# zyc00/Point-SAM

Hardware: NVIDIA H100
Metric: point-clouds/sec (N=32768, ViT-L, 512x64 groups) (higher is better)
Workload: dtype bf16x3

## Files before the change

point-sam_b200/csrc/attention_tc.cu:

```cuda
#include "psam_common.cuh"
#include "../../include/psam_b200.h"

namespace psam {

constexpr int ATT_BQ = 128;
constexpr int ATT_BKEY = 64;
constexpr int ATT_STAGES = 4;
constexpr int ATT_THREADS = 288;
constexpr int ATT_Q_TILE = 128 * 64 * 2;
constexpr int ATT_KV_TILE = 64 * 64 * 2;

template <int NCH>
struct AttSmem {
    static constexpr int Q = NCH * 2 * ATT_Q_TILE;
    static constexpr int STAGE = NCH * 2 * ATT_KV_TILE;
    static constexpr int TOTAL = Q + ATT_STAGES * STAGE + 1024;
};

struct AttnParams {
    int L, H, B;
    float scale_log2e;
    __nv_bfloat16* out_hi;
    long long out_plane, ldo, out_h, out_b;
};

__device__ __forceinline__ float ex2f(float x) {
    float e;
    asm("ex2.approx.ftz.f32 %0, %1;" : "=f"(e) : "f"(x));
    return e;
}

__device__ __forceinline__ float quad_max(float v) {
    v = fmaxf(v, __shfl_xor_sync(0xffffffffu, v, 1));
    return fmaxf(v, __shfl_xor_sync(0xffffffffu, v, 2));
}

__device__ __forceinline__ uint32_t bf16x2_bits(float lo, float hi) {
    const __nv_bfloat162 h2 = __floats2bfloat162_rn(lo, hi);
    return *reinterpret_cast<const uint32_t*>(&h2);
}

template <int NCH, int KS_LAST>
__device__ __forceinline__ void att_scores(float (&s)[32], uint32_t sq, uint32_t sk) {
#pragma unroll
    for (int i = 0; i < 32; ++i) s[i] = 0.f;
    fence_acc(s);
    wgmma_fence();
#pragma unroll
    for (int pass = 0; pass < 3; ++pass) {
#pragma unroll
        for (int ch = 0; ch < NCH; ++ch) {
            const uint64_t qd = gmma_desc_k(sq + ch * 2 * ATT_Q_TILE + (pass == 1 ? ATT_Q_TILE : 0));
            const uint64_t kd = gmma_desc_k(sk + ch * 2 * ATT_KV_TILE + (pass == 2 ? ATT_KV_TILE : 0));
#pragma unroll
            for (int k = 0; k < (ch == NCH - 1 ? KS_LAST : 4); ++k) wgmma_ss<64>(s, qd + 2 * k, kd + 2 * k, 1u);
        }
    }
    wgmma_commit();
    wgmma_wait<0>();
    fence_acc(s);
}

__device__ __forceinline__ void att_mask(float (&s)[32], int key0, int L, int lane) {
    if (key0 + ATT_BKEY <= L) return;
#pragma unroll
    for (int i = 0; i < 32; ++i)
        if (key0 + 8 * (i >> 2) + 2 * (lane & 3) + (i & 1) >= L) s[i] = __int_as_float(0xff800000);
}

template <int DH, bool TWO_PASS>
__global__ void __launch_bounds__(ATT_THREADS, 1)
attention_wgmma_kernel(const __grid_constant__ CUtensorMap tmap_q, const __grid_constant__ CUtensorMap tmap_k,
                       const __grid_constant__ CUtensorMap tmap_v, const AttnParams p) {
    constexpr int NCH = DH <= 64 ? 1 : 2;
    constexpr int KS_LAST = DH <= 64 ? 4 : (DH - 64 + 15) / 16;
    using S = AttSmem<NCH>;
    pdl_launch_dependents();
    extern __shared__ unsigned char smem_dyn[];
    __shared__ __align__(8) uint64_t q_full, kv_full[ATT_STAGES], kv_empty[ATT_STAGES];

    const uint32_t smem_base = (smem_u32(smem_dyn) + 1023u) & ~1023u;
    const uint32_t sQ = smem_base;
    const uint32_t sKV = sQ + S::Q;
    const int warp = threadIdx.x >> 5, lane = threadIdx.x & 31;
    const int q_tile = blockIdx.x, h = blockIdx.y, b = blockIdx.z;
    const int nkb = (p.L + ATT_BKEY - 1) / ATT_BKEY;

    if (warp == 8 && lane == 0) {
        tma_prefetch_desc(&tmap_q);
        tma_prefetch_desc(&tmap_k);
        tma_prefetch_desc(&tmap_v);
        mbar_init(smem_u32(&q_full), 1);
        for (int s = 0; s < ATT_STAGES; ++s) {
            mbar_init(smem_u32(&kv_full[s]), 1);
            mbar_init(smem_u32(&kv_empty[s]), 2);
        }
        fence_mbar_init();
    }
    __syncthreads();
    pdl_wait();

    const int n_items = (TWO_PASS ? 3 : 2) * nkb;
    if (warp == 8) {
        if (lane == 0) {
            const uint32_t qb = smem_u32(&q_full);
            mbar_arrive_expect_tx(qb, (uint32_t)S::Q);
            for (int ch = 0; ch < NCH; ++ch)
                tma_load_5d(sQ + ch * 2 * ATT_Q_TILE, &tmap_q, qb, 64 * ch, q_tile * ATT_BQ, 0, h, b);
            for (int i = 0; i < n_items; ++i) {
                const int s = i % ATT_STAGES;
                mbar_wait(smem_u32(&kv_empty[s]), ((uint32_t)(i / ATT_STAGES) & 1u) ^ 1u);
                const uint32_t fb = smem_u32(&kv_full[s]);
                mbar_arrive_expect_tx(fb, (uint32_t)S::STAGE);
                const int i2 = TWO_PASS ? i - nkb : i;
                const bool is_v = i2 >= 0 && (i2 & 1);
                const int blk = i2 < 0 ? i : (i2 >> 1);
                for (int ch = 0; ch < NCH; ++ch)
                    tma_load_5d(sKV + s * S::STAGE + ch * 2 * ATT_KV_TILE, is_v ? &tmap_v : &tmap_k, fb, 64 * ch, blk * ATT_BKEY, 0, h, b);
            }
        }
        return;
    }

    const int wg = warp >> 2;
    const bool leader = (warp & 3) == 0 && lane == 0;
    const uint32_t sq = sQ + wg * (ATT_Q_TILE / 2);
    const float c = p.scale_log2e;
    mbar_wait(smem_u32(&q_full), 0);
    int item = 0;
    auto acquire = [&]() {
        const int s = item % ATT_STAGES;
        mbar_wait(smem_u32(&kv_full[s]), (uint32_t)(item / ATT_STAGES) & 1u);
        return sKV + s * S::STAGE;
    };
    auto release = [&]() {
        if (leader) mbar_arrive(smem_u32(&kv_empty[item % ATT_STAGES]));
        ++item;
    };

    float m[2] = {__int_as_float(0xff800000), __int_as_float(0xff800000)};
    float s[32];
    if (TWO_PASS) {
        for (int j = 0; j < nkb; ++j) {
            att_scores<NCH, KS_LAST>(s, sq, acquire());
            release();
            att_mask(s, j * ATT_BKEY, p.L, lane);
#pragma unroll
            for (int i = 0; i < 32; ++i) m[(i >> 1) & 1] = fmaxf(m[(i >> 1) & 1], s[i]);
        }
        m[0] = quad_max(m[0]);
        m[1] = quad_max(m[1]);
    }
    float o[NCH][32];
#pragma unroll
    for (int ch = 0; ch < NCH; ++ch)
#pragma unroll
        for (int i = 0; i < 32; ++i) o[ch][i] = 0.f;
    float l[2] = {0.f, 0.f};
    for (int j = 0; j < nkb; ++j) {
        att_scores<NCH, KS_LAST>(s, sq, acquire());
        release();
        att_mask(s, j * ATT_BKEY, p.L, lane);
        if (!TWO_PASS) {
            float mb[2] = {m[0], m[1]};
#pragma unroll
            for (int i = 0; i < 32; ++i) mb[(i >> 1) & 1] = fmaxf(mb[(i >> 1) & 1], s[i]);
#pragma unroll
            for (int q = 0; q < 2; ++q) {
                mb[q] = quad_max(mb[q]);
                const float f = ex2f((m[q] - mb[q]) * c);
                l[q] *= f;
#pragma unroll
                for (int ch = 0; ch < NCH; ++ch)
#pragma unroll
                    for (int i = 0; i < 32; ++i)
                        if (((i >> 1) & 1) == q) o[ch][i] *= f;
                m[q] = mb[q];
            }
        }
        uint32_t ph[4][4], pl[4][4];
        const float nm[2] = {-m[0] * c, -m[1] * c};
#pragma unroll
        for (int kk = 0; kk < 4; ++kk) {
#pragma unroll
            for (int r = 0; r < 4; ++r) {
                const int i = 8 * kk + 2 * r, q = r & 1;
                const float e0 = ex2f(fmaf(s[i], c, nm[q])), e1 = ex2f(fmaf(s[i + 1], c, nm[q]));
                l[q] += e0 + e1;
                ph[kk][r] = bf16x2_bits(e0, e1);
                const float2 hf = __bfloat1622float2(*reinterpret_cast<const __nv_bfloat162*>(&ph[kk][r]));
                pl[kk][r] = bf16x2_bits(e0 - hf.x, e1 - hf.y);
            }
        }
        const uint32_t sv = acquire();
#pragma unroll
        for (int ch = 0; ch < NCH; ++ch) fence_acc(o[ch]);
        wgmma_fence();
#pragma unroll
        for (int ch = 0; ch < NCH; ++ch) {
            const uint64_t v_hi = gmma_desc_mn64(sv + ch * 2 * ATT_KV_TILE), v_lo = gmma_desc_mn64(sv + ch * 2 * ATT_KV_TILE + ATT_KV_TILE);
#pragma unroll
            for (int kk = 0; kk < 4; ++kk) {
                wgmma_rs_tb<64>(o[ch], ph[kk], v_hi + (uint64_t)(kk * (2048 >> 4)));
                wgmma_rs_tb<64>(o[ch], pl[kk], v_hi + (uint64_t)(kk * (2048 >> 4)));
                wgmma_rs_tb<64>(o[ch], ph[kk], v_lo + (uint64_t)(kk * (2048 >> 4)));
            }
        }
        wgmma_commit();
        wgmma_wait<0>();
#pragma unroll
        for (int ch = 0; ch < NCH; ++ch) fence_acc(o[ch]);
        release();
    }
    const int rbase = q_tile * ATT_BQ + wg * 64 + (warp & 3) * 16 + (lane >> 2);
#pragma unroll
    for (int q = 0; q < 2; ++q) {
        float lq = l[q] + __shfl_xor_sync(0xffffffffu, l[q], 1);
        lq += __shfl_xor_sync(0xffffffffu, lq, 2);
        const float inv = 1.0f / lq;
        const int row = rbase + 8 * q;
        if (row >= p.L) continue;
        __nv_bfloat16* ohi = p.out_hi + (long long)b * p.out_b + (long long)h * p.out_h + (long long)row * p.ldo;
        __nv_bfloat16* olo = ohi + p.out_plane;
#pragma unroll
        for (int ch = 0; ch < NCH; ++ch) {
#pragma unroll
            for (int g = 0; g < 8; ++g) {
                const int col = ch * 64 + 8 * g + 2 * (lane & 3);
                if (col >= DH) continue;
                __nv_bfloat16 h0, l0, h1, l1;
                split_bf16(o[ch][4 * g + 2 * q] * inv, h0, l0);
                split_bf16(o[ch][4 * g + 2 * q + 1] * inv, h1, l1);
                *reinterpret_cast<uint32_t*>(ohi + col) = pack_bf16x2(h0, h1);
                *reinterpret_cast<uint32_t*>(olo + col) = pack_bf16x2(l0, l1);
            }
        }
    }
}

int make_operand_map_ext(CUtensorMap* map, const psam_operand* op, int box_rows, int box_planes);

static int attention_setup(const psam_operand* q, const psam_operand* k, const psam_operand* v, void* out_hi, long long out_plane,
                           long long ldo, long long out_head_stride, long long out_cloud_stride, float scale, CUtensorMap* mq,
                           CUtensorMap* mk, CUtensorMap* mv, AttnParams* p, dim3* grid) {
    if (!q || !k || !v || !out_hi) return PSAM_ERR_ARG;
    const int L = q->rows, dh = q->k;
    const int H = q->nb1 > 0 ? q->nb1 : 1, B = q->nb2 > 0 ? q->nb2 : 1;
    if ((dh != 64 && dh != 88) || L <= 0) return PSAM_ERR_UNSUPPORTED;
    if (k->rows != L || v->rows != L || k->k != dh || v->k != dh) return PSAM_ERR_ARG;
    for (const psam_operand* x : {k, v})
        if ((x->nb1 > 0 ? x->nb1 : 1) != H || (x->nb2 > 0 ? x->nb2 : 1) != B) return PSAM_ERR_ARG;
    if (!(scale > 0.f) || !isfinite(scale)) return PSAM_ERR_ARG;
    if ((ldo | out_plane | out_head_stride | out_cloud_stride) & 7) return PSAM_ERR_ARG;
    int rc = make_operand_map_ext(mq, q, ATT_BQ, 2);
    if (rc) return rc;
    rc = make_operand_map_ext(mk, k, ATT_BKEY, 2);
    if (rc) return rc;
    rc = make_operand_map_ext(mv, v, ATT_BKEY, 2);
    if (rc) return rc;
    p->L = L, p->H = H, p->B = B;
    p->scale_log2e = scale * 1.4426950408889634f;
    p->out_hi = (__nv_bfloat16*)out_hi;
    p->out_plane = out_plane, p->ldo = ldo, p->out_h = out_head_stride, p->out_b = out_cloud_stride;
    *grid = dim3((unsigned)ceil_div(L, ATT_BQ), (unsigned)H, (unsigned)B);
    return PSAM_OK;
}

template <int DH, bool TWO_PASS>
static int launch_attention(const CUtensorMap& mq, const CUtensorMap& mk, const CUtensorMap& mv, const AttnParams& p, dim3 grid,
                            cudaStream_t stream) {
    auto kern = attention_wgmma_kernel<DH, TWO_PASS>;
    constexpr int smem = AttSmem<DH <= 64 ? 1 : 2>::TOTAL;
    PSAM_CUDA_TRY(cudaFuncSetAttribute(kern, cudaFuncAttributeMaxDynamicSharedMemorySize, smem));
    PSAM_CUDA_TRY(psam::launch(kern, grid, dim3(ATT_THREADS), (size_t)smem, stream, mq, mk, mv, p));
    PSAM_LAUNCH_CHECK();
    return PSAM_OK;
}

}

extern "C" int psam_attention_bf16x3(const psam_operand* q, const psam_operand* k, const psam_operand* v, void* out_hi,
                                     long long out_plane, long long ldo, long long out_head_stride,
                                     long long out_cloud_stride, float scale, cudaStream_t stream) {
    using namespace psam;
    CUtensorMap mq, mk, mv;
    AttnParams p;
    dim3 grid;
    int rc = attention_setup(q, k, v, out_hi, out_plane, ldo, out_head_stride, out_cloud_stride, scale, &mq, &mk, &mv, &p, &grid);
    if (rc) return rc;
    if (q->k == 88) return launch_attention<88, false>(mq, mk, mv, p, grid, stream);
    return launch_attention<64, false>(mq, mk, mv, p, grid, stream);
}

extern "C" int psam_attention_bf16x3_twopass(const psam_operand* q, const psam_operand* k, const psam_operand* v, void* out_hi,
                                             long long out_plane, long long ldo, long long out_head_stride,
                                             long long out_cloud_stride, float scale, cudaStream_t stream) {
    using namespace psam;
    CUtensorMap mq, mk, mv;
    AttnParams p;
    dim3 grid;
    if (q && q->k != 64) return PSAM_ERR_UNSUPPORTED;
    int rc = attention_setup(q, k, v, out_hi, out_plane, ldo, out_head_stride, out_cloud_stride, scale, &mq, &mk, &mv, &p, &grid);
    if (rc) return rc;
    return launch_attention<64, true>(mq, mk, mv, p, grid, stream);
}
```

point-sam_b200/csrc/psam_common.cuh:

```cuda
#pragma once
#include <cuda.h>
#include <cuda_bf16.h>
#include <cuda_runtime.h>
#include <stdint.h>
#include <stdlib.h>
#include <utility>

#define PSAM_OK 0
#define PSAM_ERR_ARG (-1)
#define PSAM_ERR_UNSUPPORTED (-2)

#define PSAM_CUDA_TRY(expr)                      \
    do {                                         \
        cudaError_t _e = (expr);                 \
        if (_e != cudaSuccess) return (int)_e;   \
    } while (0)

#define PSAM_LAUNCH_CHECK()                      \
    do {                                         \
        cudaError_t _e = cudaGetLastError();     \
        if (_e != cudaSuccess) return (int)_e;   \
    } while (0)

namespace psam {


__device__ __forceinline__ void pdl_launch_dependents() { asm volatile("griddepcontrol.launch_dependents;" ::: "memory"); }
__device__ __forceinline__ void pdl_wait() { asm volatile("griddepcontrol.wait;" ::: "memory"); }
__device__ __forceinline__ void pdl_prologue() {
    pdl_launch_dependents();
    pdl_wait();
}

inline bool pdl_enabled() {
    static int v = -1;
    if (v < 0) {
        const char* e = getenv("PSAM_PDL");
        v = (e && e[0] == '1') ? 1 : 0;
    }
    return v != 0;
}

template <typename... KArgs, typename... Args>
inline cudaError_t launch(void (*kernel)(KArgs...), dim3 grid, dim3 block, size_t smem, cudaStream_t stream, Args&&... args) {
    cudaLaunchConfig_t cfg = {};
    cfg.gridDim = grid;
    cfg.blockDim = block;
    cfg.dynamicSmemBytes = smem;
    cfg.stream = stream;
    cudaLaunchAttribute attr[1];
    attr[0].id = cudaLaunchAttributeProgrammaticStreamSerialization;
    attr[0].val.programmaticStreamSerializationAllowed = 1;
    cfg.attrs = attr;
    cfg.numAttrs = pdl_enabled() ? 1 : 0;
    return cudaLaunchKernelEx(&cfg, kernel, static_cast<KArgs>(std::forward<Args>(args))...);
}

__host__ __device__ inline int ceil_div(int a, int b) { return (a + b - 1) / b; }
__host__ __device__ inline long long ceil_div_ll(long long a, long long b) { return (a + b - 1) / b; }

__device__ __forceinline__ void split_bf16(float x, __nv_bfloat16& hi, __nv_bfloat16& lo) {
    hi = __float2bfloat16_rn(x);
    lo = __float2bfloat16_rn(x - __bfloat162float(hi));
}

__device__ __forceinline__ uint32_t pack_bf16x2(__nv_bfloat16 a, __nv_bfloat16 b) {
    return (uint32_t)__bfloat16_as_ushort(a) | ((uint32_t)__bfloat16_as_ushort(b) << 16);
}

__device__ __forceinline__ float gelu_erf(float x) {
    const float z = x * 0.70710678118654752440f;
    const float a = fabsf(z);
    const float t = __fdividef(1.0f, fmaf(0.3275911f, a, 1.0f));
    float p = fmaf(1.061405429f, t, -1.453152027f);
    p = fmaf(p, t, 1.421413741f);
    p = fmaf(p, t, -0.284496736f);
    p = fmaf(p, t, 0.254829592f);
    p *= t;
    const float e = __expf(-a * a);
    const float erf_abs = fmaf(-p, e, 1.0f);
    const float hx = 0.5f * x;
    return fmaf(hx, copysignf(erf_abs, z), hx);
}

__device__ __forceinline__ float silu(float x) { return x / (1.0f + __expf(-x)); }

__device__ __forceinline__ float sqdist3(float x, float y, float z, float cx, float cy, float cz) {
    const float dx = x - cx, dy = y - cy, dz = z - cz;
    return __fmaf_rn(dz, dz, __fmaf_rn(dy, dy, __fmul_rn(dx, dx)));
}

template <int NT>
__device__ __forceinline__ unsigned long long block_scan_u64(unsigned long long x, unsigned long long* sw, unsigned long long& total) {
    const int lane = threadIdx.x & 31, warp = threadIdx.x >> 5;
#pragma unroll
    for (int off = 1; off < 32; off <<= 1) {
        const unsigned long long y = __shfl_up_sync(0xffffffffu, x, off);
        if (lane >= off) x += y;
    }
    if (lane == 31) sw[warp] = x;
    __syncthreads();
    if (warp == 0) {
        unsigned long long s = lane < NT / 32 ? sw[lane] : 0ull;
#pragma unroll
        for (int off = 1; off < 32; off <<= 1) {
            const unsigned long long y = __shfl_up_sync(0xffffffffu, s, off);
            if (lane >= off) s += y;
        }
        sw[lane] = s;
    }
    __syncthreads();
    if (warp) x += sw[warp - 1];
    total = sw[NT / 32 - 1];
    __syncthreads();
    return x;
}

template <int NT>
__device__ __forceinline__ void scan_block_sums(unsigned long long* sums, int nb, unsigned long long* total) {
    __shared__ unsigned long long sw[32];
    unsigned long long carry = 0;
    for (int base = 0; base < nb; base += NT) {
        const int i = base + threadIdx.x;
        const unsigned long long v = i < nb ? sums[i] : 0ull;
        unsigned long long t;
        const unsigned long long x = block_scan_u64<NT>(v, sw, t);
        if (i < nb) sums[i] = carry + x - v;
        carry += t;
    }
    if (threadIdx.x == 0 && total) *total = carry;
}

enum Act { ACT_NONE = 0, ACT_GELU = 1, ACT_RELU = 2 };

__device__ __forceinline__ float apply_act(float x, int act) {
    if (act == ACT_GELU) return gelu_erf(x);
    if (act == ACT_RELU) return fmaxf(x, 0.0f);
    return x;
}

__device__ __forceinline__ uint32_t smem_u32(const void* p) {
    return (uint32_t)__cvta_generic_to_shared(p);
}

__device__ __forceinline__ void mbar_init(uint32_t bar, uint32_t count) {
    asm volatile("mbarrier.init.shared::cta.b64 [%0], %1;" ::"r"(bar), "r"(count));
}

__device__ __forceinline__ void fence_mbar_init() {
    asm volatile("fence.mbarrier_init.release.cluster;" ::: "memory");
}

__device__ __forceinline__ void fence_proxy_async() {
    asm volatile("fence.proxy.async.shared::cta;" ::: "memory");
}

__device__ __forceinline__ void mbar_arrive_expect_tx(uint32_t bar, uint32_t bytes) {
    asm volatile("mbarrier.arrive.expect_tx.shared::cta.b64 _, [%0], %1;" ::"r"(bar), "r"(bytes) : "memory");
}

__device__ __forceinline__ void mbar_arrive(uint32_t bar) {
    asm volatile("mbarrier.arrive.shared::cta.b64 _, [%0];" ::"r"(bar) : "memory");
}

__device__ __forceinline__ bool mbar_try_wait(uint32_t bar, uint32_t parity) {
    uint32_t ok;
    asm volatile(
        "{\n\t.reg .pred p;\n\t"
        "mbarrier.try_wait.parity.shared::cta.b64 p, [%1], %2;\n\t"
        "selp.b32 %0, 1, 0, p;\n\t}"
        : "=r"(ok)
        : "r"(bar), "r"(parity)
        : "memory");
    return ok != 0;
}

__device__ __forceinline__ void mbar_wait(uint32_t bar, uint32_t parity) {
    while (!mbar_try_wait(bar, parity)) {
    }
}

__device__ __forceinline__ void mbar_arrive_remote_release(uint32_t remote_bar) {
    asm volatile("mbarrier.arrive.release.cluster.shared::cluster.b64 _, [%0];" ::"r"(remote_bar) : "memory");
}

__device__ __forceinline__ bool mbar_try_wait_acquire_cluster(uint32_t bar, uint32_t parity) {
    uint32_t ok;
    asm volatile(
        "{\n\t.reg .pred p;\n\t"
        "mbarrier.try_wait.parity.acquire.cluster.shared::cta.b64 p, [%1], %2;\n\t"
        "selp.b32 %0, 1, 0, p;\n\t}"
        : "=r"(ok)
        : "r"(bar), "r"(parity)
        : "memory");
    return ok != 0;
}

__device__ __forceinline__ uint32_t cluster_ctarank() {
    uint32_t r;
    asm volatile("mov.u32 %0, %%cluster_ctarank;" : "=r"(r));
    return r;
}

__device__ __forceinline__ uint32_t cluster_nctarank() {
    uint32_t r;
    asm volatile("mov.u32 %0, %%cluster_nctarank;" : "=r"(r));
    return r;
}

__device__ __forceinline__ uint32_t mapa_shared(uint32_t addr, uint32_t cta) {
    uint32_t r;
    asm volatile("mapa.shared::cluster.u32 %0, %1, %2;" : "=r"(r) : "r"(addr), "r"(cta));
    return r;
}

__device__ __forceinline__ void st_cluster_v4(uint32_t addr, uint32_t a, uint32_t b, uint32_t c, uint32_t d) {
    asm volatile("st.shared::cluster.v4.u32 [%0], {%1, %2, %3, %4};" ::"r"(addr), "r"(a), "r"(b), "r"(c), "r"(d) : "memory");
}

__device__ __forceinline__ void st_cluster_u32(uint32_t addr, uint32_t a) {
    asm volatile("st.shared::cluster.u32 [%0], %1;" ::"r"(addr), "r"(a) : "memory");
}

__device__ __forceinline__ void cluster_sync_all() {
    asm volatile("barrier.cluster.arrive.release.aligned;\n\tbarrier.cluster.wait.acquire.aligned;" ::: "memory");
}

__device__ __forceinline__ void tma_prefetch_desc(const void* tmap) {
    asm volatile("prefetch.tensormap [%0];" ::"l"(tmap) : "memory");
}

__device__ __forceinline__ void tma_load_5d(uint32_t smem_dst, const void* tmap, uint32_t bar, int c0, int c1, int c2,
                                            int c3, int c4) {
    asm volatile(
        "cp.async.bulk.tensor.5d.shared::cluster.global.mbarrier::complete_tx::bytes [%0], [%1, {%3, %4, %5, %6, %7}], [%2];"
        ::"r"(smem_dst), "l"(tmap), "r"(bar), "r"(c0), "r"(c1), "r"(c2), "r"(c3), "r"(c4)
        : "memory");
}

__device__ __forceinline__ void tma_prefetch_l2_5d(const void* tmap, int c0, int c1, int c2, int c3, int c4) {
    asm volatile("cp.async.bulk.prefetch.tensor.5d.L2.global.tile [%0, {%1, %2, %3, %4, %5}];"
                 ::"l"(tmap), "r"(c0), "r"(c1), "r"(c2), "r"(c3), "r"(c4) : "memory");
}

__device__ __forceinline__ void tma_load_5d_mc(uint32_t smem_dst, const void* tmap, uint32_t bar, int c0, int c1, int c2,
                                               int c3, int c4, uint16_t cta_mask) {
    asm volatile(
        "cp.async.bulk.tensor.5d.shared::cluster.global.mbarrier::complete_tx::bytes.multicast::cluster [%0], [%1, {%3, %4, %5, %6, %7}], [%2], %8;"
        ::"r"(smem_dst), "l"(tmap), "r"(bar), "r"(c0), "r"(c1), "r"(c2), "r"(c3), "r"(c4), "h"(cta_mask)
        : "memory");
}

__device__ __forceinline__ void wgmma_fence() { asm volatile("wgmma.fence.sync.aligned;" ::: "memory"); }
__device__ __forceinline__ void wgmma_commit() { asm volatile("wgmma.commit_group.sync.aligned;" ::: "memory"); }
template <int N>
__device__ __forceinline__ void wgmma_wait() { asm volatile("wgmma.wait_group.sync.aligned %0;" ::"n"(N) : "memory"); }

template <int R>
__device__ __forceinline__ void fence_acc(float (&d)[R]) {
#pragma unroll
    for (int i = 0; i < R; ++i) asm volatile("" : "+f"(d[i])::"memory");
}

__device__ __forceinline__ uint64_t gmma_desc_sw128(uint32_t smem_addr, uint32_t lbo, uint32_t sbo) {
    uint64_t d = 0;
    d |= (uint64_t)((smem_addr & 0x3FFFFu) >> 4);
    d |= (uint64_t)((lbo >> 4) & 0x3FFFu) << 16;
    d |= (uint64_t)((sbo >> 4) & 0x3FFFu) << 32;
    d |= (uint64_t)1 << 62;
    return d;
}
__device__ __forceinline__ uint64_t gmma_desc_k(uint32_t smem_addr) { return gmma_desc_sw128(smem_addr, 16, 1024); }
__device__ __forceinline__ uint64_t gmma_desc_mn64(uint32_t smem_addr) { return gmma_desc_sw128(smem_addr, 1024, 1024); }
__device__ __forceinline__ uint64_t gmma_desc_k_sw64(uint32_t smem_addr) {
    uint64_t d = 0;
    d |= (uint64_t)((smem_addr & 0x3FFFFu) >> 4);
    d |= (uint64_t)1 << 16;
    d |= (uint64_t)(512 >> 4) << 32;
    d |= (uint64_t)2 << 62;
    return d;
}

template <int N>
__device__ __forceinline__ void wgmma_ss(float (&d)[N / 2], uint64_t adesc, uint64_t bdesc, uint32_t scale_d);
template <int N>
__device__ __forceinline__ void wgmma_rs_tb(float (&d)[N / 2], const uint32_t (&a)[4], uint64_t bdesc);

template <>
__device__ __forceinline__ void wgmma_ss<64>(float (&d)[32], uint64_t adesc, uint64_t bdesc, uint32_t scale_d) {
    asm volatile(
        "{\n\t.reg .pred p;\n\tsetp.ne.b32 p, %34, 0;\n\t"
        "wgmma.mma_async.sync.aligned.m64n64k16.f32.bf16.bf16 {%0, %1, %2, %3, %4, %5, %6, %7, %8, %9, %10, %11, %12, %13, %14, %15, %16, %17, %18, %19, %20, %21, %22, %23, %24, %25, %26, %27, %28, %29, %30, %31}, %32, %33, p, 1, 1, 0, 0;\n\t}"
        : "+f"(d[0]), "+f"(d[1]), "+f"(d[2]), "+f"(d[3]), "+f"(d[4]), "+f"(d[5]), "+f"(d[6]), "+f"(d[7]), "+f"(d[8]), "+f"(d[9]), "+f"(d[10]), "+f"(d[11]), "+f"(d[12]), "+f"(d[13]), "+f"(d[14]), "+f"(d[15]), "+f"(d[16]), "+f"(d[17]), "+f"(d[18]), "+f"(d[19]), "+f"(d[20]), "+f"(d[21]), "+f"(d[22]), "+f"(d[23]), "+f"(d[24]), "+f"(d[25]), "+f"(d[26]), "+f"(d[27]), "+f"(d[28]), "+f"(d[29]), "+f"(d[30]), "+f"(d[31])
        : "l"(adesc), "l"(bdesc), "r"(scale_d));
}
template <>
__device__ __forceinline__ void wgmma_ss<128>(float (&d)[64], uint64_t adesc, uint64_t bdesc, uint32_t scale_d) {
    asm volatile(
        "{\n\t.reg .pred p;\n\tsetp.ne.b32 p, %66, 0;\n\t"
        "wgmma.mma_async.sync.aligned.m64n128k16.f32.bf16.bf16 {%0, %1, %2, %3, %4, %5, %6, %7, %8, %9, %10, %11, %12, %13, %14, %15, %16, %17, %18, %19, %20, %21, %22, %23, %24, %25, %26, %27, %28, %29, %30, %31, %32, %33, %34, %35, %36, %37, %38, %39, %40, %41, %42, %43, %44, %45, %46, %47, %48, %49, %50, %51, %52, %53, %54, %55, %56, %57, %58, %59, %60, %61, %62, %63}, %64, %65, p, 1, 1, 0, 0;\n\t}"
        : "+f"(d[0]), "+f"(d[1]), "+f"(d[2]), "+f"(d[3]), "+f"(d[4]), "+f"(d[5]), "+f"(d[6]), "+f"(d[7]), "+f"(d[8]), "+f"(d[9]), "+f"(d[10]), "+f"(d[11]), "+f"(d[12]), "+f"(d[13]), "+f"(d[14]), "+f"(d[15]), "+f"(d[16]), "+f"(d[17]), "+f"(d[18]), "+f"(d[19]), "+f"(d[20]), "+f"(d[21]), "+f"(d[22]), "+f"(d[23]), "+f"(d[24]), "+f"(d[25]), "+f"(d[26]), "+f"(d[27]), "+f"(d[28]), "+f"(d[29]), "+f"(d[30]), "+f"(d[31]), "+f"(d[32]), "+f"(d[33]), "+f"(d[34]), "+f"(d[35]), "+f"(d[36]), "+f"(d[37]), "+f"(d[38]), "+f"(d[39]), "+f"(d[40]), "+f"(d[41]), "+f"(d[42]), "+f"(d[43]), "+f"(d[44]), "+f"(d[45]), "+f"(d[46]), "+f"(d[47]), "+f"(d[48]), "+f"(d[49]), "+f"(d[50]), "+f"(d[51]), "+f"(d[52]), "+f"(d[53]), "+f"(d[54]), "+f"(d[55]), "+f"(d[56]), "+f"(d[57]), "+f"(d[58]), "+f"(d[59]), "+f"(d[60]), "+f"(d[61]), "+f"(d[62]), "+f"(d[63])
        : "l"(adesc), "l"(bdesc), "r"(scale_d));
}
template <>
__device__ __forceinline__ void wgmma_ss<256>(float (&d)[128], uint64_t adesc, uint64_t bdesc, uint32_t scale_d) {
    asm volatile(
        "{\n\t.reg .pred p;\n\tsetp.ne.b32 p, %130, 0;\n\t"
        "wgmma.mma_async.sync.aligned.m64n256k16.f32.bf16.bf16 {%0, %1, %2, %3, %4, %5, %6, %7, %8, %9, %10, %11, %12, %13, %14, %15, %16, %17, %18, %19, %20, %21, %22, %23, %24, %25, %26, %27, %28, %29, %30, %31, %32, %33, %34, %35, %36, %37, %38, %39, %40, %41, %42, %43, %44, %45, %46, %47, %48, %49, %50, %51, %52, %53, %54, %55, %56, %57, %58, %59, %60, %61, %62, %63, %64, %65, %66, %67, %68, %69, %70, %71, %72, %73, %74, %75, %76, %77, %78, %79, %80, %81, %82, %83, %84, %85, %86, %87, %88, %89, %90, %91, %92, %93, %94, %95, %96, %97, %98, %99, %100, %101, %102, %103, %104, %105, %106, %107, %108, %109, %110, %111, %112, %113, %114, %115, %116, %117, %118, %119, %120, %121, %122, %123, %124, %125, %126, %127}, %128, %129, p, 1, 1, 0, 0;\n\t}"
        : "+f"(d[0]), "+f"(d[1]), "+f"(d[2]), "+f"(d[3]), "+f"(d[4]), "+f"(d[5]), "+f"(d[6]), "+f"(d[7]), "+f"(d[8]), "+f"(d[9]), "+f"(d[10]), "+f"(d[11]), "+f"(d[12]), "+f"(d[13]), "+f"(d[14]), "+f"(d[15]), "+f"(d[16]), "+f"(d[17]), "+f"(d[18]), "+f"(d[19]), "+f"(d[20]), "+f"(d[21]), "+f"(d[22]), "+f"(d[23]), "+f"(d[24]), "+f"(d[25]), "+f"(d[26]), "+f"(d[27]), "+f"(d[28]), "+f"(d[29]), "+f"(d[30]), "+f"(d[31]), "+f"(d[32]), "+f"(d[33]), "+f"(d[34]), "+f"(d[35]), "+f"(d[36]), "+f"(d[37]), "+f"(d[38]), "+f"(d[39]), "+f"(d[40]), "+f"(d[41]), "+f"(d[42]), "+f"(d[43]), "+f"(d[44]), "+f"(d[45]), "+f"(d[46]), "+f"(d[47]), "+f"(d[48]), "+f"(d[49]), "+f"(d[50]), "+f"(d[51]), "+f"(d[52]), "+f"(d[53]), "+f"(d[54]), "+f"(d[55]), "+f"(d[56]), "+f"(d[57]), "+f"(d[58]), "+f"(d[59]), "+f"(d[60]), "+f"(d[61]), "+f"(d[62]), "+f"(d[63]), "+f"(d[64]), "+f"(d[65]), "+f"(d[66]), "+f"(d[67]), "+f"(d[68]), "+f"(d[69]), "+f"(d[70]), "+f"(d[71]), "+f"(d[72]), "+f"(d[73]), "+f"(d[74]), "+f"(d[75]), "+f"(d[76]), "+f"(d[77]), "+f"(d[78]), "+f"(d[79]), "+f"(d[80]), "+f"(d[81]), "+f"(d[82]), "+f"(d[83]), "+f"(d[84]), "+f"(d[85]), "+f"(d[86]), "+f"(d[87]), "+f"(d[88]), "+f"(d[89]), "+f"(d[90]), "+f"(d[91]), "+f"(d[92]), "+f"(d[93]), "+f"(d[94]), "+f"(d[95]), "+f"(d[96]), "+f"(d[97]), "+f"(d[98]), "+f"(d[99]), "+f"(d[100]), "+f"(d[101]), "+f"(d[102]), "+f"(d[103]), "+f"(d[104]), "+f"(d[105]), "+f"(d[106]), "+f"(d[107]), "+f"(d[108]), "+f"(d[109]), "+f"(d[110]), "+f"(d[111]), "+f"(d[112]), "+f"(d[113]), "+f"(d[114]), "+f"(d[115]), "+f"(d[116]), "+f"(d[117]), "+f"(d[118]), "+f"(d[119]), "+f"(d[120]), "+f"(d[121]), "+f"(d[122]), "+f"(d[123]), "+f"(d[124]), "+f"(d[125]), "+f"(d[126]), "+f"(d[127])
        : "l"(adesc), "l"(bdesc), "r"(scale_d));
}
template <>
__device__ __forceinline__ void wgmma_rs_tb<64>(float (&d)[32], const uint32_t (&a)[4], uint64_t bdesc) {
    asm volatile(
        "wgmma.mma_async.sync.aligned.m64n64k16.f32.bf16.bf16 {%0, %1, %2, %3, %4, %5, %6, %7, %8, %9, %10, %11, %12, %13, %14, %15, %16, %17, %18, %19, %20, %21, %22, %23, %24, %25, %26, %27, %28, %29, %30, %31}, {%32, %33, %34, %35}, %36, 1, 1, 1, 1;"
        : "+f"(d[0]), "+f"(d[1]), "+f"(d[2]), "+f"(d[3]), "+f"(d[4]), "+f"(d[5]), "+f"(d[6]), "+f"(d[7]), "+f"(d[8]), "+f"(d[9]), "+f"(d[10]), "+f"(d[11]), "+f"(d[12]), "+f"(d[13]), "+f"(d[14]), "+f"(d[15]), "+f"(d[16]), "+f"(d[17]), "+f"(d[18]), "+f"(d[19]), "+f"(d[20]), "+f"(d[21]), "+f"(d[22]), "+f"(d[23]), "+f"(d[24]), "+f"(d[25]), "+f"(d[26]), "+f"(d[27]), "+f"(d[28]), "+f"(d[29]), "+f"(d[30]), "+f"(d[31])
        : "r"(a[0]), "r"(a[1]), "r"(a[2]), "r"(a[3]), "l"(bdesc));
}

__device__ __forceinline__ bool elect_one() {
    uint32_t pred;
    asm volatile(
        "{\n\t.reg .pred p;\n\t"
        "elect.sync _|p, 0xffffffff;\n\t"
        "selp.b32 %0, 1, 0, p;\n\t}"
        : "=r"(pred));
    return pred != 0;
}

}
```

Before: 374.8.

## Pipeline attention: overlap next QK^T with softmax, ping-pong warpgroups, register Q

Restructures the attention main loop so the next block's QK^T wgmma is issued before the current block's softmax. The two consumer warpgroups alternate tensor-core turns through named barriers, letting softmax exp work overlap MMA. For head dims up to 64, Q is loaded once into registers via ldmatrix and fed as the register operand. The change also deepens the KV ring to 5 or 6 stages, trims the last PV tile width to the actual head dim, and defers the O rescale. The cost is more register pressure and more complex barrier scheduling.

```diff
diff --git a/point-sam_b200/csrc/attention_tc.cu b/point-sam_b200/csrc/attention_tc.cu
--- a/point-sam_b200/csrc/attention_tc.cu
+++ b/point-sam_b200/csrc/attention_tc.cu
@@ -5,16 +5,18 @@
 
 constexpr int ATT_BQ = 128;
 constexpr int ATT_BKEY = 64;
-constexpr int ATT_STAGES = 4;
+constexpr int ATT_MAX_STAGES = 6;
 constexpr int ATT_THREADS = 288;
 constexpr int ATT_Q_TILE = 128 * 64 * 2;
 constexpr int ATT_KV_TILE = 64 * 64 * 2;
 
 template <int NCH>
 struct AttSmem {
+    static constexpr int STAGES = NCH == 1 ? 6 : 5;
     static constexpr int Q = NCH * 2 * ATT_Q_TILE;
     static constexpr int STAGE = NCH * 2 * ATT_KV_TILE;
-    static constexpr int TOTAL = Q + ATT_STAGES * STAGE + 1024;
+    static constexpr int TOTAL = Q + STAGES * STAGE + 1024;
+    static_assert(STAGES <= ATT_MAX_STAGES, "mbarrier arrays");
 };
 
 struct AttnParams {
@@ -40,8 +42,29 @@
     return *reinterpret_cast<const uint32_t*>(&h2);
 }
 
+template <int ID>
+__device__ __forceinline__ void named_bar_sync(int n) { asm volatile("bar.sync %0, %1;" ::"n"(ID), "r"(n) : "memory"); }
+template <int ID>
+__device__ __forceinline__ void named_bar_arrive(int n) { asm volatile("bar.arrive %0, %1;" ::"n"(ID), "r"(n) : "memory"); }
+
 template <int NCH, int KS_LAST>
-__device__ __forceinline__ void att_scores(float (&s)[32], uint32_t sq, uint32_t sk) {
+__device__ __forceinline__ void att_load_q(uint32_t (&qf)[2][NCH][4][4], uint32_t sq, int warp4, int lane) {
+    const int mi = lane >> 3, r = 16 * warp4 + (mi & 1) * 8 + (lane & 7);
+#pragma unroll
+    for (int pl = 0; pl < 2; ++pl)
+#pragma unroll
+        for (int ch = 0; ch < NCH; ++ch)
+#pragma unroll
+            for (int k = 0; k < (ch == NCH - 1 ? KS_LAST : 4); ++k) {
+                const uint32_t a = sq + ch * 2 * ATT_Q_TILE + pl * ATT_Q_TILE + r * 128 + (((2 * k + (mi >> 1)) ^ (r & 7)) << 4);
+                asm volatile("ldmatrix.sync.aligned.m8n8.x4.shared.b16 {%0, %1, %2, %3}, [%4];"
+                             : "=r"(qf[pl][ch][k][0]), "=r"(qf[pl][ch][k][1]), "=r"(qf[pl][ch][k][2]), "=r"(qf[pl][ch][k][3])
+                             : "r"(a));
+            }
+}
+
+template <int NCH, int KS_LAST>
+__device__ __forceinline__ void att_scores(float (&s)[32], const uint32_t (&qf)[2][NCH][4][4], uint32_t sq, uint32_t sk) {
 #pragma unroll
     for (int i = 0; i < 32; ++i) s[i] = 0.f;
     fence_acc(s);
@@ -50,15 +73,28 @@
     for (int pass = 0; pass < 3; ++pass) {
 #pragma unroll
         for (int ch = 0; ch < NCH; ++ch) {
+            const uint64_t kd = gmma_desc_k(sk + ch * 2 * ATT_KV_TILE + (pass == 2 ? ATT_KV_TILE : 0));
             const uint64_t qd = gmma_desc_k(sq + ch * 2 * ATT_Q_TILE + (pass == 1 ? ATT_Q_TILE : 0));
-            const uint64_t kd = gmma_desc_k(sk + ch * 2 * ATT_KV_TILE + (pass == 2 ? ATT_KV_TILE : 0));
-#pragma unroll
-            for (int k = 0; k < (ch == NCH - 1 ? KS_LAST : 4); ++k) wgmma_ss<64>(s, qd + 2 * k, kd + 2 * k, 1u);
+#pragma unroll
+            for (int k = 0; k < (ch == NCH - 1 ? KS_LAST : 4); ++k) {
+                if (NCH == 1) wgmma_rs<64>(s, qf[pass == 1][ch][k], kd + 2 * k);
+                else wgmma_ss<64>(s, qd + 2 * k, kd + 2 * k, 1u);
+            }
         }
     }
     wgmma_commit();
-    wgmma_wait<0>();
-    fence_acc(s);
+}
+
+template <int N>
+__device__ __forceinline__ void att_pv(float (&o)[32], const uint32_t (&ph)[4][4], const uint32_t (&pl)[4][4], uint32_t sv) {
+    float(&d)[N / 2] = *reinterpret_cast<float(*)[N / 2]>(&o[0]);
+    const uint64_t v_hi = gmma_desc_mn64(sv), v_lo = gmma_desc_mn64(sv + ATT_KV_TILE);
+#pragma unroll
+    for (int kk = 0; kk < 4; ++kk) {
+        wgmma_rs_tb<N>(d, ph[kk], v_hi + (uint64_t)(kk * (2048 >> 4)));
+        wgmma_rs_tb<N>(d, pl[kk], v_hi + (uint64_t)(kk * (2048 >> 4)));
+        wgmma_rs_tb<N>(d, ph[kk], v_lo + (uint64_t)(kk * (2048 >> 4)));
+    }
 }
 
 __device__ __forceinline__ void att_mask(float (&s)[32], int key0, int L, int lane) {
@@ -74,10 +110,12 @@
                        const __grid_constant__ CUtensorMap tmap_v, const AttnParams p) {
     constexpr int NCH = DH <= 64 ? 1 : 2;
     constexpr int KS_LAST = DH <= 64 ? 4 : (DH - 64 + 15) / 16;
+    constexpr int NV_LAST = DH <= 64 ? 64 : (DH - 64 + 7) / 8 * 8;
     using S = AttSmem<NCH>;
+    constexpr int STAGES = S::STAGES;
     pdl_launch_dependents();
     extern __shared__ unsigned char smem_dyn[];
-    __shared__ __align__(8) uint64_t q_full, kv_full[ATT_STAGES], kv_empty[ATT_STAGES];
+    __shared__ __align__(8) uint64_t q_full, kv_full[ATT_MAX_STAGES], kv_empty[ATT_MAX_STAGES];
 
     const uint32_t smem_base = (smem_u32(smem_dyn) + 1023u) & ~1023u;
     const uint32_t sQ = smem_base;
@@ -91,7 +129,7 @@
         tma_prefetch_desc(&tmap_k);
         tma_prefetch_desc(&tmap_v);
         mbar_init(smem_u32(&q_full), 1);
-        for (int s = 0; s < ATT_STAGES; ++s) {
+        for (int s = 0; s < STAGES; ++s) {
             mbar_init(smem_u32(&kv_full[s]), 1);
             mbar_init(smem_u32(&kv_empty[s]), 2);
         }
@@ -108,8 +146,8 @@
             for (int ch = 0; ch < NCH; ++ch)
                 tma_load_5d(sQ + ch * 2 * ATT_Q_TILE, &tmap_q, qb, 64 * ch, q_tile * ATT_BQ, 0, h, b);
             for (int i = 0; i < n_items; ++i) {
-                const int s = i % ATT_STAGES;
-                mbar_wait(smem_u32(&kv_empty[s]), ((uint32_t)(i / ATT_STAGES) & 1u) ^ 1u);
+                const int s = i % STAGES;
+                mbar_wait(smem_u32(&kv_empty[s]), ((uint32_t)(i / STAGES) & 1u) ^ 1u);
                 const uint32_t fb = smem_u32(&kv_full[s]);
                 mbar_arrive_expect_tx(fb, (uint32_t)S::STAGE);
                 const int i2 = TWO_PASS ? i - nkb : i;
@@ -124,26 +162,27 @@
 
     const int wg = warp >> 2;
     const bool leader = (warp & 3) == 0 && lane == 0;
-    const uint32_t sq = sQ + wg * (ATT_Q_TILE / 2);
     const float c = p.scale_log2e;
     mbar_wait(smem_u32(&q_full), 0);
-    int item = 0;
-    auto acquire = [&]() {
-        const int s = item % ATT_STAGES;
-        mbar_wait(smem_u32(&kv_full[s]), (uint32_t)(item / ATT_STAGES) & 1u);
-        return sKV + s * S::STAGE;
-    };
-    auto release = [&]() {
-        if (leader) mbar_arrive(smem_u32(&kv_empty[item % ATT_STAGES]));
-        ++item;
+    const uint32_t sq = sQ + wg * (ATT_Q_TILE / 2);
+    uint32_t qf[2][NCH][4][4];
+    if (NCH == 1) att_load_q<NCH, KS_LAST>(qf, sq, warp & 3, lane);
+    auto acquire = [&](int i) {
+        mbar_wait(smem_u32(&kv_full[i % STAGES]), (uint32_t)(i / STAGES) & 1u);
+        return sKV + (i % STAGES) * S::STAGE;
+    };
+    auto release = [&](int i) {
+        if (leader) mbar_arrive(smem_u32(&kv_empty[i % STAGES]));
     };
 
     float m[2] = {__int_as_float(0xff800000), __int_as_float(0xff800000)};
     float s[32];
     if (TWO_PASS) {
         for (int j = 0; j < nkb; ++j) {
-            att_scores<NCH, KS_LAST>(s, sq, acquire());
-            release();
+            att_scores<NCH, KS_LAST>(s, qf, sq, acquire(j));
+            wgmma_wait<0>();
+            fence_acc(s);
+            release(j);
             att_mask(s, j * ATT_BKEY, p.L, lane);
 #pragma unroll
             for (int i = 0; i < 32; ++i) m[(i >> 1) & 1] = fmaxf(m[(i >> 1) & 1], s[i]);
@@ -151,15 +190,16 @@
         m[0] = quad_max(m[0]);
         m[1] = quad_max(m[1]);
     }
+    const int kv0 = TWO_PASS ? nkb : 0;
     float o[NCH][32];
 #pragma unroll
     for (int ch = 0; ch < NCH; ++ch)
 #pragma unroll
         for (int i = 0; i < 32; ++i) o[ch][i] = 0.f;
     float l[2] = {0.f, 0.f};
-    for (int j = 0; j < nkb; ++j) {
-        att_scores<NCH, KS_LAST>(s, sq, acquire());
-        release();
+    float f[2] = {0.f, 0.f};
+
+    auto softmax = [&](int j) {
         att_mask(s, j * ATT_BKEY, p.L, lane);
         if (!TWO_PASS) {
             float mb[2] = {m[0], m[1]};
@@ -168,50 +208,85 @@
 #pragma unroll
             for (int q = 0; q < 2; ++q) {
                 mb[q] = quad_max(mb[q]);
-                const float f = ex2f((m[q] - mb[q]) * c);
-                l[q] *= f;
-#pragma unroll
-                for (int ch = 0; ch < NCH; ++ch)
-#pragma unroll
-                    for (int i = 0; i < 32; ++i)
-                        if (((i >> 1) & 1) == q) o[ch][i] *= f;
+                f[q] = ex2f((m[q] - mb[q]) * c);
+                l[q] *= f[q];
                 m[q] = mb[q];
             }
         }
-        uint32_t ph[4][4], pl[4][4];
         const float nm[2] = {-m[0] * c, -m[1] * c};
 #pragma unroll
+        for (int i = 0; i < 32; i += 2) {
+            const int q = (i >> 1) & 1;
+            const float e0 = ex2f(fmaf(s[i], c, nm[q])), e1 = ex2f(fmaf(s[i + 1], c, nm[q]));
+            l[q] += e0 + e1;
+            s[i] = e0;
+            s[i + 1] = e1;
+        }
+    };
+    uint32_t ph[4][4], pl[4][4];
+    auto split_p = [&]() {
+#pragma unroll
         for (int kk = 0; kk < 4; ++kk) {
 #pragma unroll
             for (int r = 0; r < 4; ++r) {
-                const int i = 8 * kk + 2 * r, q = r & 1;
-                const float e0 = ex2f(fmaf(s[i], c, nm[q])), e1 = ex2f(fmaf(s[i + 1], c, nm[q]));
-                l[q] += e0 + e1;
-                ph[kk][r] = bf16x2_bits(e0, e1);
+                const int i = 8 * kk + 2 * r;
+                ph[kk][r] = bf16x2_bits(s[i], s[i + 1]);
                 const float2 hf = __bfloat1622float2(*reinterpret_cast<const __nv_bfloat162*>(&ph[kk][r]));
-                pl[kk][r] = bf16x2_bits(e0 - hf.x, e1 - hf.y);
-            }
-        }
-        const uint32_t sv = acquire();
+                pl[kk][r] = bf16x2_bits(s[i] - hf.x, s[i + 1] - hf.y);
+            }
+        }
+    };
+    if (wg == 1) named_bar_arrive<1>(256);
+    auto turn_begin = [&]() {
+        if (wg == 0) named_bar_sync<1>(256);
+        else named_bar_sync<2>(256);
+    };
+    auto turn_end = [&](bool last) {
+        if (wg == 0) named_bar_arrive<2>(256);
+        else if (!last) named_bar_arrive<1>(256);
+    };
+
+    turn_begin();
+    att_scores<NCH, KS_LAST>(s, qf, sq, acquire(kv0));
+    turn_end(false);
+    wgmma_wait<0>();
+    fence_acc(s);
+    release(kv0);
+    softmax(0);
+    split_p();
+    auto turn = [&](int j, auto more_t) {
+        constexpr bool more = decltype(more_t)::value;
+        turn_begin();
+        if (more) att_scores<NCH, KS_LAST>(s, qf, sq, acquire(kv0 + 2 * j + 2));
+        if (!TWO_PASS) {
+#pragma unroll
+            for (int ch = 0; ch < NCH; ++ch)
+#pragma unroll
+                for (int i = 0; i < 32; ++i) o[ch][i] *= f[(i >> 1) & 1];
+        }
+        const uint32_t sv = acquire(kv0 + 2 * j + 1);
 #pragma unroll
         for (int ch = 0; ch < NCH; ++ch) fence_acc(o[ch]);
         wgmma_fence();
 #pragma unroll
-        for (int ch = 0; ch < NCH; ++ch) {
-            const uint64_t v_hi = gmma_desc_mn64(sv + ch * 2 * ATT_KV_TILE), v_lo = gmma_desc_mn64(sv + ch * 2 * ATT_KV_TILE + ATT_KV_TILE);
-#pragma unroll
-            for (int kk = 0; kk < 4; ++kk) {
-                wgmma_rs_tb<64>(o[ch], ph[kk], v_hi + (uint64_t)(kk * (2048 >> 4)));
-                wgmma_rs_tb<64>(o[ch], pl[kk], v_hi + (uint64_t)(kk * (2048 >> 4)));
-                wgmma_rs_tb<64>(o[ch], ph[kk], v_lo + (uint64_t)(kk * (2048 >> 4)));
-            }
-        }
+        for (int ch = 0; ch < NCH - 1; ++ch) att_pv<64>(o[ch], ph, pl, sv + ch * 2 * ATT_KV_TILE);
+        att_pv<NV_LAST>(o[NCH - 1], ph, pl, sv + (NCH - 1) * 2 * ATT_KV_TILE);
         wgmma_commit();
+        turn_end(!more);
+        if (more) {
+            wgmma_wait<1>();
+            fence_acc(s);
+            release(kv0 + 2 * j + 2);
+            softmax(j + 1);
+        }
         wgmma_wait<0>();
 #pragma unroll
         for (int ch = 0; ch < NCH; ++ch) fence_acc(o[ch]);
-        release();
-    }
+        release(kv0 + 2 * j + 1);
+        if (more) split_p();
+    };
+    for (int j = 0; j + 1 < nkb; ++j) turn(j, std::true_type{});
+    turn(nkb - 1, std::false_type{});
     const int rbase = q_tile * ATT_BQ + wg * 64 + (warp & 3) * 16 + (lane >> 2);
 #pragma unroll
     for (int q = 0; q < 2; ++q) {
diff --git a/point-sam_b200/csrc/psam_common.cuh b/point-sam_b200/csrc/psam_common.cuh
--- a/point-sam_b200/csrc/psam_common.cuh
+++ b/point-sam_b200/csrc/psam_common.cuh
@@ -285,6 +285,8 @@
 __device__ __forceinline__ void wgmma_ss(float (&d)[N / 2], uint64_t adesc, uint64_t bdesc, uint32_t scale_d);
 template <int N>
 __device__ __forceinline__ void wgmma_rs_tb(float (&d)[N / 2], const uint32_t (&a)[4], uint64_t bdesc);
+template <int N>
+__device__ __forceinline__ void wgmma_rs(float (&d)[N / 2], const uint32_t (&a)[4], uint64_t bdesc);
 
 template <>
 __device__ __forceinline__ void wgmma_ss<64>(float (&d)[32], uint64_t adesc, uint64_t bdesc, uint32_t scale_d) {
@@ -315,6 +317,20 @@
     asm volatile(
         "wgmma.mma_async.sync.aligned.m64n64k16.f32.bf16.bf16 {%0, %1, %2, %3, %4, %5, %6, %7, %8, %9, %10, %11, %12, %13, %14, %15, %16, %17, %18, %19, %20, %21, %22, %23, %24, %25, %26, %27, %28, %29, %30, %31}, {%32, %33, %34, %35}, %36, 1, 1, 1, 1;"
         : "+f"(d[0]), "+f"(d[1]), "+f"(d[2]), "+f"(d[3]), "+f"(d[4]), "+f"(d[5]), "+f"(d[6]), "+f"(d[7]), "+f"(d[8]), "+f"(d[9]), "+f"(d[10]), "+f"(d[11]), "+f"(d[12]), "+f"(d[13]), "+f"(d[14]), "+f"(d[15]), "+f"(d[16]), "+f"(d[17]), "+f"(d[18]), "+f"(d[19]), "+f"(d[20]), "+f"(d[21]), "+f"(d[22]), "+f"(d[23]), "+f"(d[24]), "+f"(d[25]), "+f"(d[26]), "+f"(d[27]), "+f"(d[28]), "+f"(d[29]), "+f"(d[30]), "+f"(d[31])
+        : "r"(a[0]), "r"(a[1]), "r"(a[2]), "r"(a[3]), "l"(bdesc));
+}
+template <>
+__device__ __forceinline__ void wgmma_rs<64>(float (&d)[32], const uint32_t (&a)[4], uint64_t bdesc) {
+    asm volatile(
+        "wgmma.mma_async.sync.aligned.m64n64k16.f32.bf16.bf16 {%0, %1, %2, %3, %4, %5, %6, %7, %8, %9, %10, %11, %12, %13, %14, %15, %16, %17, %18, %19, %20, %21, %22, %23, %24, %25, %26, %27, %28, %29, %30, %31}, {%32, %33, %34, %35}, %36, 1, 1, 1, 0;"
+        : "+f"(d[0]), "+f"(d[1]), "+f"(d[2]), "+f"(d[3]), "+f"(d[4]), "+f"(d[5]), "+f"(d[6]), "+f"(d[7]), "+f"(d[8]), "+f"(d[9]), "+f"(d[10]), "+f"(d[11]), "+f"(d[12]), "+f"(d[13]), "+f"(d[14]), "+f"(d[15]), "+f"(d[16]), "+f"(d[17]), "+f"(d[18]), "+f"(d[19]), "+f"(d[20]), "+f"(d[21]), "+f"(d[22]), "+f"(d[23]), "+f"(d[24]), "+f"(d[25]), "+f"(d[26]), "+f"(d[27]), "+f"(d[28]), "+f"(d[29]), "+f"(d[30]), "+f"(d[31])
+        : "r"(a[0]), "r"(a[1]), "r"(a[2]), "r"(a[3]), "l"(bdesc));
+}
+template <>
+__device__ __forceinline__ void wgmma_rs_tb<24>(float (&d)[12], const uint32_t (&a)[4], uint64_t bdesc) {
+    asm volatile(
+        "wgmma.mma_async.sync.aligned.m64n24k16.f32.bf16.bf16 {%0, %1, %2, %3, %4, %5, %6, %7, %8, %9, %10, %11}, {%12, %13, %14, %15}, %16, 1, 1, 1, 1;"
+        : "+f"(d[0]), "+f"(d[1]), "+f"(d[2]), "+f"(d[3]), "+f"(d[4]), "+f"(d[5]), "+f"(d[6]), "+f"(d[7]), "+f"(d[8]), "+f"(d[9]), "+f"(d[10]), "+f"(d[11])
         : "r"(a[0]), "r"(a[1]), "r"(a[2]), "r"(a[3]), "l"(bdesc));
 }
 
```

Result: no change. 377.4 (median of 6 runs) (+0.7%).
